# Xiaohao-Liu/EliMRec

Hardware: AMD Instinct MI355X
Metric: BPR triplets/sec (Tiktok-shape, d=128x3) (higher is better)
Workload: dtype f32; 1 GPU; tiktok-shape-synthetic; num_items=76085, train_interactions=571503, recdim=64, layer_num=3, batch_per_gpu=2048, global_batch=2048, parallelism=colshard1, graph_table=column-sharded (64 of 64 columns per rank): hops need no communication, feature_tables=replicated S_m / c, feature_dtype=f32, columns_per_gpu=64, propagation=folded, head_rows=batch, step_issue=one host call per step (csrc/program.hip): 1243 of the 1243 timed steps

## Files before the change

elimrec_amd/csrc/bwd_w.h:

```cpp
#pragma once
#include "common.h"
#include <cstdlib>

namespace elimrec {

constexpr int kMaxBatch = 8;
typedef float v16f __attribute__((ext_vector_type(16)));
#ifndef ELIMREC_BWDW_TN2
#define ELIMREC_BWDW_TN2 64
#endif
constexpr int TN1 = 64, TN2 = ELIMREC_BWDW_TN2, TRB = 32;
constexpr int BNJ = TN2 / 64, BC4 = TN2 / 4, BRP = 256 / BC4, BPS = TRB / BRP;

struct BwdProblem {
    elimrec_linear_bwd_desc d;
    int chunk_rows, chunks, t1, t2;
    int first_block;
    float *slabs, *cslabs;
};
struct BwdBatch { BwdProblem p[kMaxBatch]; int n; };

__device__ __forceinline__ void bwd_w_partial_body(const BwdBatch &batch, int block, float (*As)[TRB * TN1], float (*Bs)[TRB * TN2]) {
    const int tid = threadIdx.x, lane = tid & 63, wave = tid >> 6;
    int pi = 0;
    while (pi + 1 < batch.n && block >= batch.p[pi + 1].first_block) ++pi;
    const BwdProblem &pb = batch.p[pi];
    const int local = block - pb.first_block;
    const int n1_tiles = pb.t1, n2_tiles = pb.t2;
    const int chunk = local / (n1_tiles * n2_tiles);
    const int tile = local - chunk * (n1_tiles * n2_tiles);
    const int tile_y = tile / n2_tiles, tile_z = tile - tile_y * n2_tiles;
    const float *__restrict__ A = pb.d.d_A;
    const float *__restrict__ B = pb.d.d_B;
    const int32_t *__restrict__ row_index = pb.d.d_row_index;
    const int32_t *__restrict__ range = pb.d.d_range;
    const int64_t lda = pb.d.lda, ldb = pb.d.ldb, R = pb.d.R;
    const int n1 = pb.d.n1, n2 = pb.d.n2, chunk_rows = pb.chunk_rows;
    float *__restrict__ slabs = pb.slabs;
    float *__restrict__ colsum_slabs = pb.d.d_colsum ? pb.cslabs : nullptr;
    const float *__restrict__ cw = pb.d.d_colsum ? pb.d.d_colsum_weight : nullptr;
    int64_t rb = 0, re = R;
    if (range) { rb = range[0]; re = range[1]; }
    const int64_t r0 = rb + (int64_t)chunk * chunk_rows;
    const int64_t r1 = (r0 + chunk_rows < re) ? r0 + chunk_rows : re;
    const int i_base = tile_y * TN1, j_base = tile_z * TN2;

    const int a_row = tid >> 4, a_c4 = tid & 15;
    const int b_row = tid / BC4, b_c4 = tid % BC4;
    const bool a_col_ok = (i_base + a_c4 * 4) < n1;
    const bool b_col_ok = (j_base + b_c4 * 4) < n2;
    float4 ra[2], rbv[BPS];
    float rw = 1.f, rw_cur = 1.f;
    auto load_block = [&](int64_t row0) {
        if (cw && tid < TRB) {
            const int64_t r = row0 + tid;
            rw = r < r1 ? cw[row_index ? (int64_t)row_index[r] : r] : 0.f;
        }
#pragma unroll
        for (int p = 0; p < 2; ++p) {
            const int64_t r = row0 + a_row + 16 * p;
            ra[p] = (a_col_ok && r < r1) ? *reinterpret_cast<const float4 *>(A + r * lda + i_base + a_c4 * 4)
                                         : make_float4(0.f, 0.f, 0.f, 0.f);
        }
#pragma unroll
        for (int p = 0; p < BPS; ++p) {
            const int64_t r = row0 + b_row + BRP * p;
            float4 v = make_float4(0.f, 0.f, 0.f, 0.f);
            if (b_col_ok && r < r1) {
                const int64_t br = row_index ? (int64_t)row_index[r] : r;
                v = *reinterpret_cast<const float4 *>(B + br * ldb + j_base + b_c4 * 4);
            }
            rbv[p] = v;
        }
    };
    auto store_block = [&](int buf) {
        rw_cur = rw;
#pragma unroll
        for (int p = 0; p < 2; ++p)
            *reinterpret_cast<float4 *>(&As[buf][(a_row + 16 * p) * TN1 + a_c4 * 4]) = ra[p];
#pragma unroll
        for (int p = 0; p < BPS; ++p)
            *reinterpret_cast<float4 *>(&Bs[buf][(b_row + BRP * p) * TN2 + b_c4 * 4]) = rbv[p];
    };

    const int wi = (wave & 1) * 32, wj = (wave >> 1) * (TN2 / 2);
    const int li = lane & 31, lk = lane >> 5;
    const bool wave_on = (j_base + wj) < n2;
    const bool half1_on = BNJ > 1 && (j_base + wj + 32) < n2;
    v16f acc0 = {0}, acc1 = {0};
    float csum = 0.f;
    int buf = 0;
    if (r0 < r1) {
        load_block(r0);
        store_block(0);
    }
    __syncthreads();
    for (int64_t row0 = r0; row0 < r1; row0 += TRB) {
        const bool more = (row0 + TRB) < r1;
        if (more) load_block(row0 + TRB);
        const float *as = As[buf], *bs = Bs[buf];
        if (wave_on) {
#pragma unroll
            for (int kk = 0; kk < TRB; kk += 2) {
                const float a = as[(kk + lk) * TN1 + wi + li];
                const float b0 = bs[(kk + lk) * TN2 + wj + li];
                acc0 = __builtin_amdgcn_mfma_f32_32x32x2f32(a, b0, acc0, 0, 0, 0);
                if (BNJ > 1) {
                    const float b1 = bs[(kk + lk) * TN2 + wj + (BNJ > 1 ? 32 : 0) + li];
                    acc1 = __builtin_amdgcn_mfma_f32_32x32x2f32(a, b1, acc1, 0, 0, 0);
                }
            }
        }
        if (colsum_slabs && tid < TN1) {
            if (cw) {
#pragma unroll
                for (int k = 0; k < TRB; ++k)
                    csum += as[k * TN1 + tid] * __builtin_bit_cast(float, __builtin_amdgcn_readlane(__builtin_bit_cast(int, rw_cur), k));
            } else {
#pragma unroll 8
                for (int k = 0; k < TRB; ++k) csum += as[k * TN1 + tid];
            }
        }
        if (more) store_block(buf ^ 1);
        __syncthreads();
        buf ^= 1;
    }
    const int n1_pad = n1_tiles * TN1, n2_pad = n2_tiles * TN2;
    float *slab = slabs + (size_t)chunk * n1_pad * n2_pad;
    if (wave_on) {
#pragma unroll
        for (int r = 0; r < 16; ++r) {
            const int row = i_base + wi + (r & 3) + 8 * (r >> 2) + 4 * (lane >> 5);
            slab[(size_t)row * n2_pad + j_base + wj + li] = acc0[r];
            if (half1_on) slab[(size_t)row * n2_pad + j_base + wj + 32 + li] = acc1[r];
        }
    }
    if (colsum_slabs && tile_z == 0 && tid < TN1) colsum_slabs[(size_t)chunk * n1_pad + i_base + tid] = csum;
}

__device__ __forceinline__ float slab_lane_sum(const float *src, size_t stride, int chunks, int q) {
    float s = 0.f;
    int c = q;
    for (; c + 12 < chunks; c += 16) {
        const float v0 = src[(size_t)c * stride], v1 = src[(size_t)(c + 4) * stride];
        const float v2 = src[(size_t)(c + 8) * stride], v3 = src[(size_t)(c + 12) * stride];
        s += v0; s += v1; s += v2; s += v3;
    }
    for (; c < chunks; c += 4) s += src[(size_t)c * stride];
    return s;
}

__device__ __forceinline__ void reduce_slabs_body(const BwdBatch &batch, int bx, int by) {
    const BwdProblem &pb = batch.p[by];
    const int n1 = pb.d.n1, n2 = pb.d.n2;
    const int n1_pad = pb.t1 * TN1, n2_pad = pb.t2 * TN2;
    const int gid = bx * 256 + (int)threadIdx.x;
    const int idx = gid >> 2, q = gid & 3;
    const int total = n1 * n2;
    int64_t rows = pb.d.d_range ? (int64_t)pb.d.d_range[1] - pb.d.d_range[0] : pb.d.R;
    if (rows < 0) rows = 0;
    const int chunks = (int)((rows + pb.chunk_rows - 1) / pb.chunk_rows);
    const float *src = nullptr;
    size_t stride = 0;
    float *dst = nullptr;
    if (idx < total) {
        const int i = idx / n2, j = idx - i * n2;
        src = pb.slabs + (size_t)i * n2_pad + j;
        stride = (size_t)n1_pad * n2_pad;
        dst = pb.d.d_out + (int64_t)i * pb.d.ldo + j;
    } else if (pb.d.d_colsum && idx < total + n1) {
        src = pb.cslabs + (idx - total);
        stride = (size_t)n1_pad;
        dst = pb.d.d_colsum + (idx - total);
    }
    float s = src ? slab_lane_sum(src, stride, chunks, q) : 0.f;
    s += __shfl_xor(s, 1, 64);
    s += __shfl_xor(s, 2, 64);
    if (src && q == 0) *dst = pb.d.accumulate ? (*dst + s) : s;
}


struct FoldSpan {
    const float *p_in;
    float *p_out, *m, *v, *copy_dst;
    float step_size, inv_sqrt_bc2;
};
struct FoldProblem {
    const float *slabs, *cslabs;
    const int32_t *range;
    float *out, *colsum;
    int64_t R, ldo;
    int chunk_rows, n1, n2, n1_pad, n2_pad, accumulate;
    FoldSpan w, b;
};
struct FoldBatch { FoldProblem p[kMaxBatch]; int n, gx; };

__device__ __forceinline__ void reduce_adam_body(const FoldBatch &batch, int bx, int by, float beta1, float beta2, float eps, float wd) {
    const FoldProblem &pb = batch.p[by];
    const int gid = bx * 256 + (int)threadIdx.x;
    const int idx = gid >> 2, q = gid & 3;
    const int total = pb.n1 * pb.n2;
    int64_t rows = pb.range ? (int64_t)pb.range[1] - pb.range[0] : pb.R;
    if (rows < 0) rows = 0;
    const int chunks = (int)((rows + pb.chunk_rows - 1) / pb.chunk_rows);
    const bool is_w = idx < total, is_b = !is_w && pb.cslabs && idx < total + pb.n1;
    const float *src = nullptr;
    size_t stride = 0;
    int64_t at = 0;
    if (is_w) {
        const int i = idx / pb.n2, j = idx - i * pb.n2;
        src = pb.slabs + (size_t)i * pb.n2_pad + j;
        stride = (size_t)pb.n1_pad * pb.n2_pad;
        at = (int64_t)i * pb.ldo + j;
    } else if (is_b) {
        src = pb.cslabs + (idx - total);
        stride = (size_t)pb.n1_pad;
        at = idx - total;
    }
    float s = src ? slab_lane_sum(src, stride, chunks, q) : 0.f;
    s += __shfl_xor(s, 1, 64);
    s += __shfl_xor(s, 2, 64);
    if (!src || q != 0) return;
    float *dst = (is_w ? pb.out : pb.colsum) + at;
    const float g = pb.accumulate ? (*dst + s) : s;
    *dst = g;
    const float *p_in = is_w ? pb.w.p_in : pb.b.p_in;
    if (!p_in) return;
    float *p_out = is_w ? pb.w.p_out : pb.b.p_out, *m = is_w ? pb.w.m : pb.b.m, *v = is_w ? pb.w.v : pb.b.v;
    float *copy_dst = is_w ? pb.w.copy_dst : pb.b.copy_dst;
    const float step_size = is_w ? pb.w.step_size : pb.b.step_size, inv_sqrt_bc2 = is_w ? pb.w.inv_sqrt_bc2 : pb.b.inv_sqrt_bc2;
    const float pi = p_in[at];
    if (copy_dst) copy_dst[at] = pi;
    const float gi = fmaf(wd, pi, g);
    const float mo = m[at];
    const float mi = mo + (1.f - beta1) * (gi - mo);
    const float vi = fmaf(1.f - beta2, gi * gi, beta2 * v[at]);
    const float denom = sqrtf(vi) * inv_sqrt_bc2 + eps;
    m[at] = mi;
    v[at] = vi;
    p_out[at] = pi - step_size * (mi / denom);
}


static inline void bwd_w_dims(int64_t R, int n1, int n2, int &chunk_rows, int &chunks, int &t1, int &t2) {
    const int tiles = ((n1 + TN1 - 1) / TN1) * ((n2 + TN2 - 1) / TN2);
    static int target = 0;
    if (!target) target = 480;
    int64_t want = (R * tiles + target - 1) / target;
    want = (want + TRB - 1) / TRB * TRB;
    chunk_rows = (int)(want < 64 ? 64 : (want > 512 ? 512 : want));
    chunks = (int)((R + chunk_rows - 1) / chunk_rows);
    if (chunks < 1) chunks = 1;
    t1 = (n1 + TN1 - 1) / TN1;
    t2 = (n2 + TN2 - 1) / TN2;
}

static inline size_t bwd_w_bytes(int64_t R, int n1, int n2) {
    int cr, chunks, t1, t2;
    bwd_w_dims(R, n1, n2, cr, chunks, t1, t2);
    return align_up(((size_t)chunks * t1 * TN1 * t2 * TN2 + (size_t)chunks * t1 * TN1) * sizeof(float), 256);
}


static inline int bwd_w_build_batch(const elimrec_linear_bwd_desc *descs, int n, void *d_workspace, BwdBatch &batch, int &blocks,
                                    int &max_out) {
    batch.n = n;
    char *ws = (char *)d_workspace;
    blocks = 0; max_out = 0;
    for (int i = 0; i < n; ++i) {
        const elimrec_linear_bwd_desc &d = descs[i];
        ELIMREC_REQUIRE(d.d_A && d.d_B && d.d_out, "linear_bwd_w: null pointer");
        ELIMREC_REQUIRE(d.R >= 0 && d.n1 > 0 && d.n2 > 0, "linear_bwd_w: bad shape");
        ELIMREC_REQUIRE(d.n1 % 4 == 0 && d.n2 % 4 == 0 && d.lda % 4 == 0 && d.ldb % 4 == 0,
                        "linear_bwd_w: n1, n2, lda, ldb must be multiples of 4");
        ELIMREC_REQUIRE(((uintptr_t)d.d_A % 16) == 0 && ((uintptr_t)d.d_B % 16) == 0,
                        "linear_bwd_w: A and B must be 16-byte aligned");
        BwdProblem &pb = batch.p[i];
        pb.d = d;
        bwd_w_dims(d.R, d.n1, d.n2, pb.chunk_rows, pb.chunks, pb.t1, pb.t2);
        pb.first_block = blocks;
        blocks += pb.chunks * pb.t1 * pb.t2;
        pb.slabs = (float *)ws;
        pb.cslabs = pb.slabs + (size_t)pb.chunks * pb.t1 * TN1 * pb.t2 * TN2;
        ws += bwd_w_bytes(d.R, d.n1, d.n2);
        const int out_elems = d.n1 * d.n2 + (d.d_colsum ? d.n1 : 0);
        if (out_elems > max_out) max_out = out_elems;
    }
    return 0;
}

static inline size_t bwd_w_batched_bytes(const elimrec_linear_bwd_desc *descs, int n) {
    size_t total = 0;
    for (int i = 0; i < n; ++i) total += bwd_w_bytes(descs[i].R, descs[i].n1, descs[i].n2);
    return total;
}

}
```

elimrec_amd/csrc/gemm.hip:

```cpp
#include "common.h"
#include "merge_rows.h"
#include "bwd_w.h"
#include <cstdlib>

namespace elimrec {

typedef float v16f __attribute__((ext_vector_type(16)));

constexpr int FBN = 64, FBK = 16, FLD = FBK + 1;

struct FwdBatch { elimrec_linear_desc p[kMaxBatch]; };

template <int BM, int PD>
__global__ __launch_bounds__(256) void linear_fwd_kernel(FwdBatch batch) {
    const elimrec_linear_desc &pd = batch.p[blockIdx.z];
    const float *__restrict__ A = pd.d_A;
    const float *__restrict__ W = pd.d_W;
    const float *__restrict__ bias = pd.d_bias;
    float *__restrict__ C = pd.d_C;
    const float *__restrict__ rowscale = pd.d_rowscale;
    const float *__restrict__ addm = pd.d_add;
    const int32_t *__restrict__ row_index = pd.d_row_index;
    const int64_t lda = pd.lda, ldw = pd.ldw, ldc = pd.ldc, ldadd = pd.ldadd;
    const int64_t row_lo = pd.d_row_range ? (int64_t)max(pd.d_row_range[0], 0) : 0;
    const int64_t M = pd.d_row_range ? (int64_t)min((int64_t)pd.d_row_range[1], pd.M) : pd.M;
    const int N = pd.N, K = pd.K;
    const bool relu = pd.act == 1;
    const int n0 = blockIdx.y * FBN;
    const int64_t n_tiles = M > row_lo ? (M - row_lo + BM - 1) / BM : 0;
    if ((int64_t)blockIdx.x >= n_tiles || n0 >= N) return;
    __shared__ float As[2][BM * FLD];
    __shared__ float Bs[2][FBN * FLD];
    constexpr int KP4 = FBK / 4;
    constexpr int RPP = 256 / KP4;
    constexpr int AP = BM / RPP;
    constexpr int BP = FBN / RPP;
    const int tid = threadIdx.x;
    const int lane = tid & 63;
    const int wave = tid >> 6;
    const int lr = tid / KP4;
    const int lc = (tid % KP4) * 4;
    const int wrow = (BM == 128) ? wave * 32 : (wave & 1) * 32;
    const int wcol = (BM == 128) ? 0 : (wave >> 1) * 32;
    const int chunks = (K + FBK - 1) / FBK;
    const int64_t my_tiles = (n_tiles - blockIdx.x + gridDim.x - 1) / gridDim.x;
    const int64_t G = my_tiles * chunks;

    v16f acc0 = {0}, acc1 = {0};
    const int ai = lane & 31, ak = lane >> 5;
    float4 ra[PD][AP], rb[PD][BP];
    auto load_chunk = [&](int64_t g, float4 (&qa)[AP], float4 (&qb)[BP]) {
        const int64_t m0 = row_lo + ((int64_t)blockIdx.x + (g / chunks) * gridDim.x) * BM;
        const int k0 = (int)(g % chunks) * FBK;
        const bool kin = (k0 + lc) < K;
#pragma unroll
        for (int i = 0; i < AP; ++i) {
            const int64_t gr = m0 + lr + RPP * i;
            const int64_t sr = (row_index && gr < M) ? (int64_t)row_index[gr] : gr;
            qa[i] = (kin && gr < M) ? *reinterpret_cast<const float4 *>(A + sr * lda + k0 + lc)
                                    : make_float4(0.f, 0.f, 0.f, 0.f);
        }
#pragma unroll
        for (int i = 0; i < BP; ++i) {
            const int gn = n0 + lr + RPP * i;
            qb[i] = (kin && gn < N) ? *reinterpret_cast<const float4 *>(W + (int64_t)gn * ldw + k0 + lc)
                                    : make_float4(0.f, 0.f, 0.f, 0.f);
        }
    };
    auto store_chunk = [&](int buf, const float4 (&qa)[AP], const float4 (&qb)[BP]) {
#pragma unroll
        for (int i = 0; i < AP; ++i) {
            float *dst = &As[buf][(lr + RPP * i) * FLD + lc];
            dst[0] = qa[i].x; dst[1] = qa[i].y; dst[2] = qa[i].z; dst[3] = qa[i].w;
        }
#pragma unroll
        for (int i = 0; i < BP; ++i) {
            float *dst = &Bs[buf][(lr + RPP * i) * FLD + lc];
            dst[0] = qb[i].x; dst[1] = qb[i].y; dst[2] = qb[i].z; dst[3] = qb[i].w;
        }
    };
    const int col0 = n0 + wcol + (lane & 31);
    const int col1 = col0 + 32;
    const float bias0 = (bias && col0 < N) ? bias[col0] : 0.f;
    const float bias1 = (BM == 128 && bias && col1 < N) ? bias[col1] : 0.f;

#pragma unroll
    for (int j = 0; j < PD; ++j)
        if (j < G) load_chunk(j, ra[j], rb[j]);
    int buf = 0;
    for (int64_t g0 = 0; g0 < G; g0 += PD) {
#pragma unroll
        for (int j = 0; j < PD; ++j) {
            const int64_t g = g0 + j;
            if (g >= G) break;
            store_chunk(buf, ra[j], rb[j]);
            __syncthreads();
            if (g + PD < G) load_chunk(g + PD, ra[j], rb[j]);
            const float *ap = &As[buf][(wrow + ai) * FLD + ak];
            const float *bp0 = &Bs[buf][(wcol + ai) * FLD + ak];
            const float *bp1 = &Bs[buf][(32 + ai) * FLD + ak];
#pragma unroll
            for (int kk = 0; kk < FBK; kk += 2) {
                const float a = ap[kk];
                const float b0 = bp0[kk];
                acc0 = __builtin_amdgcn_mfma_f32_32x32x2f32(a, b0, acc0, 0, 0, 0);
                if (BM == 128) {
                    const float b1 = bp1[kk];
                    acc1 = __builtin_amdgcn_mfma_f32_32x32x2f32(a, b1, acc1, 0, 0, 0);
                }
            }
            if ((int)(g % chunks) == chunks - 1) {
                const int64_t m0 = row_lo + ((int64_t)blockIdx.x + (g / chunks) * gridDim.x) * BM;
#pragma unroll
                for (int r = 0; r < 16; ++r) {
                    const int64_t row = m0 + wrow + (r & 3) + 8 * (r >> 2) + 4 * (lane >> 5);
                    if (row < M) {
                        const int64_t sr = row_index ? (int64_t)row_index[row] : row;
                        const float rs = rowscale ? rowscale[sr] : 1.f;
                        if (col0 < N) {
                            const float v = acc0[r] + rs * bias0 + (addm ? addm[sr * ldadd + col0] : 0.f);
                            C[row * ldc + col0] = relu ? fmaxf(v, 0.f) : v;
                        }
                        if (BM == 128 && col1 < N) {
                            const float v = acc1[r] + rs * bias1 + (addm ? addm[sr * ldadd + col1] : 0.f);
                            C[row * ldc + col1] = relu ? fmaxf(v, 0.f) : v;
                        }
                    }
                }
                acc0 = (v16f){0};
                acc1 = (v16f){0};
            }
            buf ^= 1;
        }
    }
}

__global__ __launch_bounds__(256) void linear_bwd_w_partial_kernel(BwdBatch batch) {
    __shared__ float As[2][TRB * TN1];
    __shared__ float Bs[2][TRB * TN2];
    bwd_w_partial_body(batch, (int)blockIdx.x, As, Bs);
}

__global__ __launch_bounds__(256) void linear_bwd_w_merge_kernel(BwdBatch batch, MergeArgs mg, int bw_blocks, int merge_blocks,
                                                                 int merge_first) {
    __shared__ float As[2][TRB * TN1];
    __shared__ float Bs[2][TRB * TN2];
    int b = (int)blockIdx.x;
    bool merge;
    if (merge_first) { merge = b < merge_blocks; if (!merge) b -= merge_blocks; }
    else { merge = b >= bw_blocks; if (merge) b -= bw_blocks; }
    if (merge) {
        int *s_beg = reinterpret_cast<int *>(&Bs[0][0]);
        slab_merge_rows_body(mg, b, s_beg, s_beg + kSlabMaxRanks, reinterpret_cast<uint32_t *>(&As[0][0]));
        return;
    }
    bwd_w_partial_body(batch, b, As, Bs);
}

__global__ void reduce_slabs_kernel(BwdBatch batch) { reduce_slabs_body(batch, (int)blockIdx.x, (int)blockIdx.y); }

}

using namespace elimrec;

extern "C" int elimrec_linear_fwd_batched(const elimrec_linear_desc *descs, int n, void *stream) {
    ELIMREC_REQUIRE(descs && n >= 1 && n <= kMaxBatch, "linear_fwd_batched: 1..%d problems", kMaxBatch);
    FwdBatch batch;
    int64_t max_tiles_m = 0;
    int max_tiles_n = 0;
    for (int i = 0; i < n; ++i) {
        const elimrec_linear_desc &d = descs[i];
        ELIMREC_REQUIRE(d.d_A && d.d_W && d.d_C, "linear_fwd: null pointer");
        ELIMREC_REQUIRE(d.M >= 0 && d.N > 0 && d.K > 0, "linear_fwd: bad shape M=%lld N=%d K=%d", (long long)d.M, d.N, d.K);
        ELIMREC_REQUIRE(d.K % 4 == 0 && d.lda % 4 == 0 && d.ldw % 4 == 0, "linear_fwd: K, lda, ldw must be multiples of 4");
        ELIMREC_REQUIRE(d.act == 0 || d.act == 1, "linear_fwd: unknown activation %d", d.act);
        ELIMREC_REQUIRE(((uintptr_t)d.d_A % 16) == 0 && ((uintptr_t)d.d_W % 16) == 0, "linear_fwd: A and W must be 16-byte aligned");
        batch.p[i] = d;
        if (d.M > max_tiles_m) max_tiles_m = d.M;
        const int tn = (d.N + FBN - 1) / FBN;
        if (tn > max_tiles_n) max_tiles_n = tn;
    }
    if (max_tiles_m == 0) return 0;
    const int tile_rows = 64;
    const int wg_budget = 1 << 30;
    int64_t per_problem = (wg_budget + (int64_t)n * max_tiles_n - 1) / ((int64_t)n * max_tiles_n);
    if (tile_rows == 128) {
        const int64_t tiles = (max_tiles_m + 127) / 128;
        dim3 grid((unsigned)(tiles < per_problem ? tiles : per_problem), (unsigned)max_tiles_n, (unsigned)n);
        hipLaunchKernelGGL((linear_fwd_kernel<128, 1>), grid, dim3(256), 0, (hipStream_t)stream, batch);
    } else {
        const int64_t tiles = (max_tiles_m + 63) / 64;
        dim3 grid((unsigned)(tiles < per_problem ? tiles : per_problem), (unsigned)max_tiles_n, (unsigned)n);
        const int depth = 0;
        const int64_t wgs = (int64_t)grid.x * grid.y * grid.z;
        const int pd = depth > 0 ? depth : (wgs <= 768 ? 8 : 1);
        if (pd >= 8) hipLaunchKernelGGL((linear_fwd_kernel<64, 8>), grid, dim3(256), 0, (hipStream_t)stream, batch);
        else if (pd >= 4) hipLaunchKernelGGL((linear_fwd_kernel<64, 4>), grid, dim3(256), 0, (hipStream_t)stream, batch);
        else hipLaunchKernelGGL((linear_fwd_kernel<64, 1>), grid, dim3(256), 0, (hipStream_t)stream, batch);
    }
    ELIMREC_LAUNCH_CHECK("linear_fwd");
    return 0;
}

extern "C" int elimrec_linear_fwd(const float *d_A, int64_t lda, const float *d_W, int64_t ldw,
                                  const float *d_bias, float *d_C, int64_t ldc, int64_t M, int N, int K,
                                  void *stream) {
    elimrec_linear_desc d = {d_A, lda, d_W, ldw, d_bias, d_C, ldc, M, N, K, nullptr, nullptr, 0, nullptr, nullptr, 0};
    return elimrec_linear_fwd_batched(&d, 1, stream);
}

extern "C" size_t elimrec_linear_bwd_w_workspace(int64_t R, int n1, int n2) { return bwd_w_bytes(R, n1, n2); }

extern "C" size_t elimrec_linear_bwd_w_batched_workspace(const elimrec_linear_bwd_desc *descs, int n) {
    size_t total = 0;
    for (int i = 0; i < n; ++i) total += bwd_w_bytes(descs[i].R, descs[i].n1, descs[i].n2);
    return total;
}

static int linear_bwd_w_batched_impl(const elimrec_linear_bwd_desc *descs, int n, void *d_workspace, size_t workspace_bytes,
                                     const MergeArgs *mg, int defer_reduce, void *stream) {
    ELIMREC_REQUIRE(descs && n >= 1 && n <= kMaxBatch, "linear_bwd_w_batched: 1..%d problems", kMaxBatch);
    ELIMREC_REQUIRE(d_workspace, "linear_bwd_w: null workspace");
    if (workspace_bytes < elimrec_linear_bwd_w_batched_workspace(descs, n)) {
        set_error("linear_bwd_w: workspace too small (%zu < %zu)", workspace_bytes,
                  elimrec_linear_bwd_w_batched_workspace(descs, n));
        return ELIMREC_E_WORKSPACE;
    }
    BwdBatch batch;
    int blocks = 0, max_out = 0, rc;
    if ((rc = bwd_w_build_batch(descs, n, d_workspace, batch, blocks, max_out))) return rc;
    hipStream_t s = (hipStream_t)stream;
    if (mg) {
        const int merge_blocks = (int)((mg->N + mg->chunk - 1) / mg->chunk);
        static int merge_first = -1;
        if (merge_first < 0) { const char *e = getenv("ELIMREC_MERGE_FIRST"); merge_first = e ? atoi(e) : 1; }
        hipLaunchKernelGGL(linear_bwd_w_merge_kernel, dim3(blocks + merge_blocks), dim3(256), 0, s, batch, *mg, blocks, merge_blocks,
                           merge_first);
    } else {
        hipLaunchKernelGGL(linear_bwd_w_partial_kernel, dim3(blocks), dim3(256), 0, s, batch);
    }
    ELIMREC_LAUNCH_CHECK("linear_bwd_w_partial");
    if (defer_reduce) return 0;
    hipLaunchKernelGGL(reduce_slabs_kernel, dim3((4 * max_out + 255) / 256, n), dim3(256), 0, s, batch);
    ELIMREC_LAUNCH_CHECK("reduce_slabs");
    return 0;
}

extern "C" int elimrec_linear_bwd_w_reduce(const elimrec_linear_bwd_desc *descs, int n, void *d_workspace, size_t workspace_bytes,
                                           void *stream) {
    ELIMREC_REQUIRE(descs && n >= 1 && n <= kMaxBatch, "linear_bwd_w_reduce: 1..%d problems", kMaxBatch);
    ELIMREC_REQUIRE(d_workspace && workspace_bytes >= bwd_w_batched_bytes(descs, n), "linear_bwd_w_reduce: workspace");
    BwdBatch batch;
    int blocks = 0, max_out = 0, rc;
    if ((rc = bwd_w_build_batch(descs, n, d_workspace, batch, blocks, max_out))) return rc;
    hipLaunchKernelGGL(reduce_slabs_kernel, dim3((4 * max_out + 255) / 256, n), dim3(256), 0, (hipStream_t)stream, batch);
    ELIMREC_LAUNCH_CHECK("reduce_slabs");
    return 0;
}

extern "C" int elimrec_linear_bwd_w_batched(const elimrec_linear_bwd_desc *descs, int n, void *d_workspace,
                                            size_t workspace_bytes, void *stream) {
    return linear_bwd_w_batched_impl(descs, n, d_workspace, workspace_bytes, nullptr, 0, stream);
}

extern "C" int elimrec_linear_bwd_w_batched_merge(const elimrec_linear_bwd_desc *descs, int n, void *d_workspace,
                                                  size_t workspace_bytes, const float *d_rows, const int32_t *d_keys, int world,
                                                  int64_t R, int64_t U, int64_t I, int ns, int w, int M, float *d_SrcA,
                                                  float *d_SrcB, uint32_t *d_mask, int defer_reduce, void *stream) {
    if (!d_rows) return linear_bwd_w_batched_impl(descs, n, d_workspace, workspace_bytes, nullptr, defer_reduce, stream);
    ELIMREC_REQUIRE(M >= 0, "linear_bwd_w_batched_merge: M >= 0");
    ELIMREC_REQUIRE(d_keys && d_SrcA && d_SrcB && d_mask, "linear_bwd_w_batched_merge: null pointer");
    ELIMREC_REQUIRE(world >= 1 && world <= kSlabMaxRanks && R >= 1 && R < INT32_MAX, "linear_bwd_w_batched_merge: 1..%d ranks", kSlabMaxRanks);
    ELIMREC_REQUIRE(ns >= 1 && w >= 4 && (w & (w - 1)) == 0, "linear_bwd_w_batched_merge: bad slab geometry (ns=%d, w=%d)", ns, w);
    const int64_t N = U + I;
    int sh = 0;
    while ((4 << sh) < w) ++sh;
    MergeArgs mg = {d_rows, d_keys, world, (int)R, U, N, ns * (w / 4), w / 4, sh, merge_rows_chunk(N), M, d_SrcA, d_SrcB, d_mask, 0};
    ELIMREC_REQUIRE(mg.chunk / 32 <= kMergeSeenWords, "linear_bwd_w_batched_merge: %lld rows are more than the fused launch takes "
                    "(call elimrec_slab_merge_rows)", (long long)N);
    return linear_bwd_w_batched_impl(descs, n, d_workspace, workspace_bytes, N > 0 ? &mg : nullptr, defer_reduce, stream);
}

extern "C" int elimrec_linear_bwd_w(const float *d_A, int64_t lda, const float *d_B, int64_t ldb,
                                    const int32_t *d_row_index, const int32_t *d_range, int64_t R, int n1, int n2,
                                    float *d_out, int64_t ldo, float *d_colsum, int accumulate, void *d_workspace,
                                    size_t workspace_bytes, void *stream) {
    elimrec_linear_bwd_desc d = {d_A, lda, d_B, ldb, d_row_index, d_range, R, n1, n2, d_out, ldo, d_colsum, accumulate, nullptr};
    return elimrec_linear_bwd_w_batched(&d, 1, d_workspace, workspace_bytes, stream);
}
```

Measured before the change: 7.423 million triplets/s.

## Compute two adjacent B column tiles per block in backward weight-gradient kernel

Each block of the weight-gradient partial kernel now covers two neighbouring 64-column B tiles, so its A tile is loaded once and reused for both. The two B shared-memory buffers, which were the double buffer, now hold the two tiles. Staging therefore becomes register prefetch with two barriers per step instead of shared-memory double buffering. Launch bounds also request 5 blocks per CU. This halves the block count and the repeated A loads, but adds a synchronisation per step and more register pressure.

```diff
diff --git a/elimrec_amd/csrc/bwd_w.h b/elimrec_amd/csrc/bwd_w.h
--- a/elimrec_amd/csrc/bwd_w.h
+++ b/elimrec_amd/csrc/bwd_w.h
@@ -6,11 +6,9 @@
 
 constexpr int kMaxBatch = 8;
 typedef float v16f __attribute__((ext_vector_type(16)));
-#ifndef ELIMREC_BWDW_TN2
-#define ELIMREC_BWDW_TN2 64
-#endif
-constexpr int TN1 = 64, TN2 = ELIMREC_BWDW_TN2, TRB = 32;
-constexpr int BNJ = TN2 / 64, BC4 = TN2 / 4, BRP = 256 / BC4, BPS = TRB / BRP;
+constexpr int TN1 = 64, TN2 = 64, TRB = 32;
+constexpr int ZT = 2;
+constexpr int BC4 = TN2 / 4, BRP = 256 / BC4, BPS = TRB / BRP;
 
 struct BwdProblem {
     elimrec_linear_bwd_desc d;
@@ -20,16 +18,18 @@
 };
 struct BwdBatch { BwdProblem p[kMaxBatch]; int n; };
 
+struct BwdStage { float4 a[2], b[ZT][BPS]; float w; };
 __device__ __forceinline__ void bwd_w_partial_body(const BwdBatch &batch, int block, float (*As)[TRB * TN1], float (*Bs)[TRB * TN2]) {
+    static_assert(ZT == 2 && TN2 == 64, "two B tiles share the two Bs stages");
     const int tid = threadIdx.x, lane = tid & 63, wave = tid >> 6;
     int pi = 0;
     while (pi + 1 < batch.n && block >= batch.p[pi + 1].first_block) ++pi;
     const BwdProblem &pb = batch.p[pi];
     const int local = block - pb.first_block;
-    const int n1_tiles = pb.t1, n2_tiles = pb.t2;
-    const int chunk = local / (n1_tiles * n2_tiles);
-    const int tile = local - chunk * (n1_tiles * n2_tiles);
-    const int tile_y = tile / n2_tiles, tile_z = tile - tile_y * n2_tiles;
+    const int n1_tiles = pb.t1, n2_tiles = pb.t2, n2_pairs = (n2_tiles + ZT - 1) / ZT;
+    const int chunk = local / (n1_tiles * n2_pairs);
+    const int tile = local - chunk * (n1_tiles * n2_pairs);
+    const int tile_y = tile / n2_pairs, pair_z = tile - tile_y * n2_pairs;
     const float *__restrict__ A = pb.d.d_A;
     const float *__restrict__ B = pb.d.d_B;
     const int32_t *__restrict__ row_index = pb.d.d_row_index;
@@ -37,78 +37,83 @@
     const int64_t lda = pb.d.lda, ldb = pb.d.ldb, R = pb.d.R;
     const int n1 = pb.d.n1, n2 = pb.d.n2, chunk_rows = pb.chunk_rows;
     float *__restrict__ slabs = pb.slabs;
-    float *__restrict__ colsum_slabs = pb.d.d_colsum ? pb.cslabs : nullptr;
-    const float *__restrict__ cw = pb.d.d_colsum ? pb.d.d_colsum_weight : nullptr;
+    float *__restrict__ colsum_slabs = (pb.d.d_colsum && pair_z == 0) ? pb.cslabs : nullptr;
+    const float *__restrict__ cw = colsum_slabs ? pb.d.d_colsum_weight : nullptr;
     int64_t rb = 0, re = R;
     if (range) { rb = range[0]; re = range[1]; }
     const int64_t r0 = rb + (int64_t)chunk * chunk_rows;
     const int64_t r1 = (r0 + chunk_rows < re) ? r0 + chunk_rows : re;
-    const int i_base = tile_y * TN1, j_base = tile_z * TN2;
+    const int i_base = tile_y * TN1, j_base = pair_z * ZT * TN2;
+    const bool tile1 = pair_z * ZT + 1 < n2_tiles;
 
     const int a_row = tid >> 4, a_c4 = tid & 15;
     const int b_row = tid / BC4, b_c4 = tid % BC4;
     const bool a_col_ok = (i_base + a_c4 * 4) < n1;
-    const bool b_col_ok = (j_base + b_c4 * 4) < n2;
-    float4 ra[2], rbv[BPS];
-    float rw = 1.f, rw_cur = 1.f;
-    auto load_block = [&](int64_t row0) {
+    const bool b_col_ok0 = (j_base + b_c4 * 4) < n2;
+    const bool b_col_ok1 = tile1 && (j_base + TN2 + b_c4 * 4) < n2;
+    BwdStage P;
+    P.w = 1.f;
+    float rw_cur = 1.f;
+    auto load_block = [&](BwdStage &g, int64_t row0) {
         if (cw && tid < TRB) {
             const int64_t r = row0 + tid;
-            rw = r < r1 ? cw[row_index ? (int64_t)row_index[r] : r] : 0.f;
+            g.w = r < r1 ? cw[row_index ? (int64_t)row_index[r] : r] : 0.f;
         }
 #pragma unroll
         for (int p = 0; p < 2; ++p) {
             const int64_t r = row0 + a_row + 16 * p;
-            ra[p] = (a_col_ok && r < r1) ? *reinterpret_cast<const float4 *>(A + r * lda + i_base + a_c4 * 4)
-                                         : make_float4(0.f, 0.f, 0.f, 0.f);
+            g.a[p] = (a_col_ok && r < r1) ? *reinterpret_cast<const float4 *>(A + r * lda + i_base + a_c4 * 4)
+                                          : make_float4(0.f, 0.f, 0.f, 0.f);
         }
 #pragma unroll
         for (int p = 0; p < BPS; ++p) {
             const int64_t r = row0 + b_row + BRP * p;
-            float4 v = make_float4(0.f, 0.f, 0.f, 0.f);
-            if (b_col_ok && r < r1) {
+            float4 v0 = make_float4(0.f, 0.f, 0.f, 0.f), v1 = v0;
+            if ((b_col_ok0 || b_col_ok1) && r < r1) {
                 const int64_t br = row_index ? (int64_t)row_index[r] : r;
-                v = *reinterpret_cast<const float4 *>(B + br * ldb + j_base + b_c4 * 4);
+                const float *src = B + br * ldb + j_base + b_c4 * 4;
+                if (b_col_ok0) v0 = *reinterpret_cast<const float4 *>(src);
+                if (b_col_ok1) v1 = *reinterpret_cast<const float4 *>(src + TN2);
             }
-            rbv[p] = v;
+            g.b[0][p] = v0;
+            g.b[1][p] = v1;
         }
     };
-    auto store_block = [&](int buf) {
-        rw_cur = rw;
+    auto store_block = [&](const BwdStage &g, int abuf) {
+        rw_cur = g.w;
 #pragma unroll
         for (int p = 0; p < 2; ++p)
-            *reinterpret_cast<float4 *>(&As[buf][(a_row + 16 * p) * TN1 + a_c4 * 4]) = ra[p];
-#pragma unroll
-        for (int p = 0; p < BPS; ++p)
-            *reinterpret_cast<float4 *>(&Bs[buf][(b_row + BRP * p) * TN2 + b_c4 * 4]) = rbv[p];
+            *reinterpret_cast<float4 *>(&As[abuf][(a_row + 16 * p) * TN1 + a_c4 * 4]) = g.a[p];
+#pragma unroll
+        for (int p = 0; p < BPS; ++p) {
+            *reinterpret_cast<float4 *>(&Bs[0][(b_row + BRP * p) * TN2 + b_c4 * 4]) = g.b[0][p];
+            if (tile1) *reinterpret_cast<float4 *>(&Bs[1][(b_row + BRP * p) * TN2 + b_c4 * 4]) = g.b[1][p];
+        }
     };
 
     const int wi = (wave & 1) * 32, wj = (wave >> 1) * (TN2 / 2);
     const int li = lane & 31, lk = lane >> 5;
-    const bool wave_on = (j_base + wj) < n2;
-    const bool half1_on = BNJ > 1 && (j_base + wj + 32) < n2;
+    const bool wave_on0 = (j_base + wj) < n2;
+    const bool wave_on1 = tile1 && (j_base + TN2 + wj) < n2;
     v16f acc0 = {0}, acc1 = {0};
     float csum = 0.f;
-    int buf = 0;
-    if (r0 < r1) {
-        load_block(r0);
-        store_block(0);
-    }
-    __syncthreads();
-    for (int64_t row0 = r0; row0 < r1; row0 += TRB) {
-        const bool more = (row0 + TRB) < r1;
-        if (more) load_block(row0 + TRB);
-        const float *as = As[buf], *bs = Bs[buf];
-        if (wave_on) {
+    auto multiply = [&](int abuf) {
+        const float *as = As[abuf], *bs0 = Bs[0], *bs1 = Bs[1];
+        if (wave_on1) {
 #pragma unroll
             for (int kk = 0; kk < TRB; kk += 2) {
                 const float a = as[(kk + lk) * TN1 + wi + li];
-                const float b0 = bs[(kk + lk) * TN2 + wj + li];
+                const float b0 = bs0[(kk + lk) * TN2 + wj + li];
+                const float b1 = bs1[(kk + lk) * TN2 + wj + li];
                 acc0 = __builtin_amdgcn_mfma_f32_32x32x2f32(a, b0, acc0, 0, 0, 0);
-                if (BNJ > 1) {
-                    const float b1 = bs[(kk + lk) * TN2 + wj + (BNJ > 1 ? 32 : 0) + li];
-                    acc1 = __builtin_amdgcn_mfma_f32_32x32x2f32(a, b1, acc1, 0, 0, 0);
-                }
+                acc1 = __builtin_amdgcn_mfma_f32_32x32x2f32(a, b1, acc1, 0, 0, 0);
+            }
+        } else if (wave_on0) {
+#pragma unroll
+            for (int kk = 0; kk < TRB; kk += 2) {
+                const float a = as[(kk + lk) * TN1 + wi + li];
+                const float b0 = bs0[(kk + lk) * TN2 + wj + li];
+                acc0 = __builtin_amdgcn_mfma_f32_32x32x2f32(a, b0, acc0, 0, 0, 0);
             }
         }
         if (colsum_slabs && tid < TN1) {
@@ -121,21 +126,34 @@
                 for (int k = 0; k < TRB; ++k) csum += as[k * TN1 + tid];
             }
         }
-        if (more) store_block(buf ^ 1);
+    };
+    if (r0 < r1) {
+        load_block(P, r0);
+        store_block(P, 0);
+    }
+    __syncthreads();
+    int buf = 0;
+    for (int64_t row0 = r0; row0 < r1; row0 += TRB) {
+        const bool more = (row0 + TRB) < r1;
+        if (more) load_block(P, row0 + TRB);
+        multiply(buf);
+        if (!more) break;
+        __syncthreads();
+        store_block(P, buf ^ 1);
         __syncthreads();
         buf ^= 1;
     }
     const int n1_pad = n1_tiles * TN1, n2_pad = n2_tiles * TN2;
     float *slab = slabs + (size_t)chunk * n1_pad * n2_pad;
-    if (wave_on) {
+    if (wave_on0) {
 #pragma unroll
         for (int r = 0; r < 16; ++r) {
             const int row = i_base + wi + (r & 3) + 8 * (r >> 2) + 4 * (lane >> 5);
             slab[(size_t)row * n2_pad + j_base + wj + li] = acc0[r];
-            if (half1_on) slab[(size_t)row * n2_pad + j_base + wj + 32 + li] = acc1[r];
-        }
-    }
-    if (colsum_slabs && tile_z == 0 && tid < TN1) colsum_slabs[(size_t)chunk * n1_pad + i_base + tid] = csum;
+            if (wave_on1) slab[(size_t)row * n2_pad + j_base + TN2 + wj + li] = acc1[r];
+        }
+    }
+    if (colsum_slabs && tid < TN1) colsum_slabs[(size_t)chunk * n1_pad + i_base + tid] = csum;
 }
 
 __device__ __forceinline__ float slab_lane_sum(const float *src, size_t stride, int chunks, int q) {
@@ -279,7 +297,7 @@
         pb.d = d;
         bwd_w_dims(d.R, d.n1, d.n2, pb.chunk_rows, pb.chunks, pb.t1, pb.t2);
         pb.first_block = blocks;
-        blocks += pb.chunks * pb.t1 * pb.t2;
+        blocks += pb.chunks * pb.t1 * ((pb.t2 + ZT - 1) / ZT);
         pb.slabs = (float *)ws;
         pb.cslabs = pb.slabs + (size_t)pb.chunks * pb.t1 * TN1 * pb.t2 * TN2;
         ws += bwd_w_bytes(d.R, d.n1, d.n2);
diff --git a/elimrec_amd/csrc/gemm.hip b/elimrec_amd/csrc/gemm.hip
--- a/elimrec_amd/csrc/gemm.hip
+++ b/elimrec_amd/csrc/gemm.hip
@@ -135,7 +135,7 @@
     }
 }
 
-__global__ __launch_bounds__(256) void linear_bwd_w_partial_kernel(BwdBatch batch) {
+__global__ __launch_bounds__(256, 5) void linear_bwd_w_partial_kernel(BwdBatch batch) {
     __shared__ float As[2][TRB * TN1];
     __shared__ float Bs[2][TRB * TN2];
     bwd_w_partial_body(batch, (int)blockIdx.x, As, Bs);
```

After: 7.500 million triplets/s, median of 6. 1.01x the previous value.
